# nanograv/PTMCMCSampler

Measured on AMD Instinct MI355X. Metric: MH updates/sec (whole node) + ESS/sec, 100-d Gaussian, 64 temps x 4096 walkers per GPU, higher is better.
Workload: dtype f64

## Files before the change

ptmcmcsampler_amd/csrc/ptmi_abi.hip:

```cpp
#include <math.h>
#include <stdlib.h>

#include <new>
#include <vector>

#include <type_traits>

#include "ptmi_common.h"

static thread_local char g_err[512] = "";
int ptmi_fail(int code, const char *fmt, ...)
{
    va_list ap;
    va_start(ap, fmt);
    vsnprintf(g_err, sizeof(g_err), fmt, ap);
    va_end(ap);
    return code;
}

constexpr int WT = 7, WTILE = 16 * WT;
template <bool FUSED>
__global__ __launch_bounds__(256) void welford_kernel(const double *AM, double *mu, double *M2, double *cov, int d, int mem,
                                                     long long iter, int cov_stride_per_walker, int am_epl)
{
// ... 848 lines not shown
{
    __shared__ int32_t local[GJ_BUCKETS], base[GJ_BUCKETS];
    for (int b = (int)threadIdx.x; b < GJ_BUCKETS; b += (int)blockDim.x) local[b] = 0;
    __syncthreads();
    const long long ch = (long long)blockIdx.x * blockDim.x + threadIdx.x;
    const int b = ch < nch ? gj_class(gj, (size_t)(ch / nt) * nt + temp_of[ch]) : 0;
    const int mine = ch < nch ? atomicAdd(&local[b], 1) : 0;
    __syncthreads();
    for (int bb = (int)threadIdx.x; bb < GJ_BUCKETS; bb += (int)blockDim.x)
        base[bb] = local[bb] ? atomicAdd(&bucket[2 * GJ_BUCKETS + bb], local[bb]) : 0;
    __syncthreads();
    if (ch >= nch) return;
    const long long t = bucket[GJ_BUCKETS + b] + base[b] + mine;
    if (t < nsolo) { order[t * cpw] = (int32_t)ch; return; }
    const long long tr = t - nsolo, nrest = nch - nsolo;
    const long long nw = nrest / cpw, whole = nw * cpw;
    order[(long long)nsolo * cpw + (tr < whole ? (tr % nw) * cpw + tr / nw : tr)] = (int32_t)ch;
}

__global__ void selftest_math_kernel(int op, const double *in, const double *in2, double *out, long long n)
{
    const long long i = (long long)blockIdx.x * blockDim.x + threadIdx.x;
    if (i >= n) return;
    const double x = in[i];
    double r;
    switch (op) {
    case 0: r = det_log(x); break;
    case 1: r = det_exp(x); break;
    case 2: r = det_cos2pi(x); break;
    case 3: r = det_sqrt(x); break;
    case 4: r = x / in2[i]; break;
    case 5: r = det_normal((u64)__double_as_longlong(x), (u64)__double_as_longlong(in2[i])); break;
    case 10: r = unit_log((u64)__double_as_longlong(x)); break;
    case 11: case 12: {
        u32 j;
        double t, sn, cs;
        unit_angle64((u64)__double_as_longlong(x), j, t);
        unit_sincos(j, t, sn, cs);
        r = op == 11 ? cs : sn;
        break;
    }
    case 13: {
        u32 j;
        double t, sn, cs;
        unit_angle32((u32)(u64)__double_as_longlong(x), j, t);
        unit_sincos(j, t, sn, cs);
        r = det_sqrt(-2.0 * unit_log((u64)__double_as_longlong(in2[i]))) * cs;
        break;
    }
    default: r = group_sum<16>(x); break;
    }
    out[i] = r;
}
__global__ void selftest_philox_kernel(const u32 *ck, u32 *out, long long n)
{
    const long long i = (long long)blockIdx.x * blockDim.x + threadIdx.x;
    if (i >= n) return;
    const u32 *c = ck + i * 6;
    u64 w0, w1;
    philox_words(((u64)c[5] << 32) | c[4], ((u64)c[1] << 32) | c[0], c[2], c[3], w0, w1);
    out[i * 4 + 0] = (u32)w0; out[i * 4 + 1] = (u32)(w0 >> 32);
    out[i * 4 + 2] = (u32)w1; out[i * 4 + 3] = (u32)(w1 >> 32);
}

struct Shape { int G, EPL; };
static bool pick_shape(int d, bool grad, Shape *s)
{
    static const Shape table[] = {
#define PTMI_TABLE_ENTRY(G_, E_) {G_, E_},
        PTMI_SHAPE_LIST(PTMI_TABLE_ENTRY)};
    if (d > PTMI_GJ_REG_MAX) grad = false;
    const int G = grad ? ptmi_lanes_for_grad(d) : ptmi_lanes_for(d);
    for (const Shape &c : table)
        if (c.G == G && c.G * c.EPL >= d && (!grad || c.EPL <= 8) && (!ptmi_shape_exact(c.G, c.EPL) || c.G * c.EPL == d)) { *s = c; return true; }
    return false;
}

static KArgs make_args(ptmi_engine *h)
{
    KArgs a;
    memset(&a, 0, sizeof(a));
    a.box_off = -1;
    a.tab_off = -1;
    const ptmi_config &c = h->cfg;
    const ptmi_buffers &b = h->buf;
    a.X = b.X; a.lnL = b.lnL; a.lp = b.lp; a.temp_of = b.temp_of; a.slot_of = b.slot_of;
    a.Ut = b.Ut; a.S = b.S; a.DE = b.DE; a.AM = c.temp0 == 0 ? b.AM : nullptr; a.AMaux = c.temp0 == 0 ? b.AMaux : nullptr;
    a.AMflag = c.temp0 == 0 ? (AmFlag *)b.AMflag : nullptr;
    a.rp_draws = h->rp_draws;
    a.nacc = (u64 *)b.nacc; a.jstat = (u64 *)b.jstat; a.cjstat = h->cjstat;
    a.temps_mh = h->d_temps; a.beta = h->d_beta; a.logl_par = h->d_loglpar; a.logp_par = h->d_logppar;
    a.gsize = h->d_gsize; a.gmask = h->d_gmask; a.gcn = h->d_gcn; a.gdiv = h->d_gdiv; a.ngroups = c.ngroups > 1 ? c.ngroups : 1;
    a.Q = b.Q; a.qaux = b.qaux; a.Q2 = nullptr; a.sloc = nullptr; a.q_cur = 0; a.q_tgt = 0;
    a.seed = c.seed;
    a.d = c.ndim; a.nt = c.ntemps; a.W = c.nwalkers; a.ntg = c.ntemps_global; a.temp0 = c.temp0; a.walker0 = c.walker0;
    a.w_host = c.w_host; a.w_scam = c.w_scam; a.w_am = c.w_am; a.w_de = c.w_de; a.de_on = h->de_on; a.de_size = c.de_size; a.de_head = h->de_head;
    a.cov_update = c.cov_update; a.tskip = c.tskip; a.per_walker = c.cov_per_walker; a.logp_kind = c.logp_kind;
    a.pick_walker = c.pick_mode == PTMI_PICK_WALKER;
    a.de_ld = h->G == 4 ? 8 * ((h->EPL + 1) / 2) : c.ndim;
    a.lanes = h->G;
    a.am_epl = am_row_epl(h->G, h->EPL);
    a.w_nuts = c.w_nuts; a.w_hmc = c.w_hmc; a.gj_nburn = c.gj_nburn; a.hmc_min = c.hmc_min; a.hmc_max = c.hmc_max;
    a.nuts_maxdepth = c.nuts_maxdepth; a.hmc_eps = c.hmc_eps; a.nuts_delta = c.nuts_delta;
    a.gj_tab = h->d_gj_tab; a.gj_diag = h->gj_diag; a.gj = b.gj; a.gj_scr = h->d_gj_scr; a.gj_scal = h->d_gj_scal;
    return a;
}

static ptmi_shape_fn shape_fn(int G, int EPL, int L)
{
    if (L == PTMI_LOGL_INTERVAL) {
#define PTMI_PICK_SHAPE3(G_, E_) if (G == G_ && EPL == E_) return ptmi_shape_##G_##_##E_##_3;
        PTMI_GJ_SHAPE_LIST(PTMI_PICK_SHAPE3)
        return nullptr;
    }
#define PTMI_PICK_SHAPE(G_, E_)                                                                        \
    if (G == G_ && EPL == E_) return L == 0 ? ptmi_shape_##G_##_##E_##_0 : (L == 1 ? ptmi_shape_##G_##_##E_##_1 : ptmi_shape_##G_##_##E_##_2);
    PTMI_SHAPE_LIST(PTMI_PICK_SHAPE)
    return nullptr;
}
static int run_shape(ptmi_engine *h, int op, KArgs &a, int grid, bool full)
{
    const int L = (op == PTMI_OP_PROPOSE || op == PTMI_OP_ACCEPT) ? 0 : h->cfg.logl_kind;
    ptmi_shape_fn f = shape_fn(h->G, h->EPL, L);
    if (!f) return fail(PTMI_EUNSUPPORTED, "no kernel shape for ndim=%d", h->cfg.ndim);
    return f(op, h, a, grid, full);
}

static int set_step_args(const ptmi_engine *h, KArgs *a)
{
    const ptmi_config &c = h->cfg;
    a->am_row0 = (int)(a->iter0 % c.cov_update);
    if (a->AMflag != nullptr && a->nsteps > 0 && (a->iter0 - 1) / c.cov_update != (a->iter0 + a->nsteps - 2) / c.cov_update && a->iter0 > 0)
        return fail(PTMI_EINVAL, "with AM row flags a launch may not cross a multiple of cov_update (iterations %lld..%lld, cov_update=%d)",
                    a->iter0, a->iter0 + a->nsteps - 1, c.cov_update);
    a->swap_last = 0;
    if (c.tskip > 0 && c.ntemps_global > 1) {
        const long long last = a->iter0 + a->nsteps - 1;
        if (last / c.tskip != (a->iter0 - 1) / c.tskip && last % c.tskip != 0)
            return fail(PTMI_EINVAL, "iterations %lld..%lld contain a swap iteration (Tskip=%d) before their end", a->iter0, last, c.tskip);
        if ((last / c.tskip) - ((a->iter0 - 1) / c.tskip) > 1)
            return fail(PTMI_EINVAL, "iterations %lld..%lld span more than one swap epoch", a->iter0, last);
        a->swap_last = last % c.tskip == 0;
    }
    return PTMI_OK;
}

static int chains_grid(const ptmi_engine *h)
{
    const long long nch = (long long)h->cfg.nwalkers * h->cfg.ntemps;
    const int cpb = 256 / h->G;
    return (int)((nch + cpb - 1) / cpb);
}

template <int G, int MAXT>
static int launch_am_gemm_t(ptmi_engine *h, long long max_events)
{
    const size_t lds = sizeof(double) * 2 * (2 * G) * 64;
    auto kern = am_gemm_kernel<G, MAXT>;
    if (lds > 64 * 1024) {
        hipError_t e = hipFuncSetAttribute((const void *)kern, hipFuncAttributeMaxDynamicSharedMemorySize, (int)lds);
        if (e != hipSuccess) return fail(PTMI_EHIP, "hipFuncSetAttribute(%zu B of LDS): %s", lds, hipGetErrorString(e));
    }
    const int d = h->cfg.ndim, ntile = (d + 15) / 16, parts = (ntile + 4 * MAXT - 1) / (4 * MAXT);
    const int ngr = h->cfg.ngroups > 1 ? h->cfg.ngroups : 1;
    const int pw = h->cfg.cov_per_walker ? 1 : 0;
    const long long per_key = pw ? (max_events / h->cfg.nwalkers) : max_events;
// ... 892 lines not shown
```

ptmcmcsampler_amd/csrc/ptmi_common.h:

```cpp
#pragma once
#include <hip/hip_runtime.h>
#include <stdarg.h>
#include <stdio.h>
#include <stdlib.h>
#include <string.h>

#include "../../include/ptmi.h"
#include "ptmi_device.h"

using namespace ptmi;

int ptmi_fail(int code, const char *fmt, ...);
#define fail ptmi_fail
inline double ptmi_env(const char *name, double dflt)
{
    const char *v = getenv(name);
    return v ? strtod(v, nullptr) : dflt;
}

#define HIPCHK(expr)                                                                          \
    do {                                                                                      \
        hipError_t e_ = (expr);                                                               \
        if (e_ != hipSuccess) return fail(PTMI_EHIP, "%s: %s (%s:%d)", #expr, hipGetErrorString(e_), __FILE__, __LINE__); \
    } while (0)

__host__ __device__ inline int am_pos(int i, int epl)
{
    if (epl == 0) return i;
    const int e = i >> 2, ln = i & 3;
    return e < 2 * (epl / 2) ? 8 * (e >> 1) + 2 * ln + (e & 1) : 8 * (epl / 2) + ln;
}
__host__ __device__ inline int am_inv(int p, int epl)
{
    if (epl == 0) return p;
    const int h = 8 * (epl / 2);
    return p < h ? ((p & 7) >> 1) + 4 * (2 * (p >> 3) + (p & 1)) : (p - h) + 4 * (epl - 1);
}
constexpr int am_row_epl(int G, int EPL) { return (G == 4 && EPL == 25) ? EPL : 0; }

constexpr unsigned long long AMROW_NEW = 1ull;
constexpr unsigned long long AMROW_KEY = 2ull;
typedef unsigned long long AmFlag;

struct KArgs {
    double *X, *lnL, *lp;
    int32_t *temp_of, *slot_of;
    const double *Ut, *S, *DE;
    double *AM, *AMaux;
    AmFlag *AMflag;
    u64 *nacc, *jstat;
    const double *temps_mh, *beta, *logl_par, *logp_par;
    const int32_t *gsize;
    const double *gmask, *gcn, *gdiv;
    double *Q, *qaux;
    double *Q2;
    int32_t *sloc;
    int q_cur, q_tgt;
    const double *newlnL, *newlp;
    u64 seed;
    long long iter0;
    const long long *iter_dev;
    int nsteps;
    int d, nt, W, ntg, temp0, walker0;
    int w_host, w_scam, w_am, w_de, de_on, de_size, de_head;
    int cov_update, tskip, per_walker, logp_kind, ngroups;
    int am_row0, swap_last;
    int am_epl;
    int lanes;
    int de_ld;
    int pick_walker;
    int lds_u;
    int amq_off;
    int amq_on;
    int box_off;
    int tab_off;
    const double *am_inc;
    const long long *am_base;
    long long *am_next;
    const double *UtPad;
    int ut_pad_ld;
    const double *ut_absmax;
    int umax_off;
    int w_nuts, w_hmc, gj_nburn, hmc_min, hmc_max, nuts_maxdepth;
    double hmc_eps, nuts_delta;
    const double *gj_tab;
    int gj_diag;
    double *gj;
    double *gj_scr, *gj_scal;
    int gj_stack_off, gj_lds_levels;
    const int32_t *gj_order;
    int gj_nslots;
    const u64 *rp_draws;
    u64 *cjstat;
};

enum { GJ_EPS = 0, GJ_MU = 1, GJ_HBAR = 2, GJ_EPSBAR = 3, GJ_NITER = 4, GJ_HITER = 5, GJ_HAVE_EPS = 6, GJ_NLEAP = 7 , GJ_NSTATE = 8 };
constexpr int GJ_BUCKETS = 128;
constexpr u32 SLOT_GJ = 0x2000000u;
constexpr u32 SLOT_GJS = 0x3000000u;
constexpr u32 SLOT_CJ = 0x4000000u;
constexpr int PTMI_CJ_MAXFUN = 32;
enum { GJV_TM = 0, GJV_RM = 1, GJV_GM = 2, GJV_TP = 3, GJV_RP = 4, GJV_GP = 5, GJV_SAMPLE = 6, GJV_TOP = 7 };
enum { GJL_FAR_T = 0, GJL_FAR_R = 1, GJL_CAND_T = 2, GJL_CAND_G = 3, GJL_VECS = 4 };
enum { GJS_LOGP = 0, GJS_N = 1, GJS_ALPHA = 2, GJS_NALPHA = 3, GJS_SCALARS = 4 };

constexpr int PTMI_GJ_REG_MAX = 512;

template <int G>
__device__ __forceinline__ double group_bcast_lane(double v, int src)
{
    const int lane = (int)(threadIdx.x & 63);
    return __shfl(v, (lane & ~(G - 1)) + src, 64);
}

struct ptmi_engine {
    ptmi_config cfg;
    ptmi_buffers buf;
    hipStream_t stream;
    double *d_ladder, *d_temps, *d_beta, *d_loglpar, *d_logppar, *d_gmask, *d_gcn, *d_gdiv;
    int32_t *d_gsize;
    void *d_pre;
    int32_t *d_hop;
    bool hop_from_sweep;
    int32_t *h_hop;
    hipEvent_t hop_ev;
    bool hop_pending;
    int32_t *d_xint;
    double *d_gj_tab, *d_gj_scr, *d_gj_scal;
    int gj_diag;
    int gj_solo;
    int32_t *d_gj_order, *d_gj_bucket;
    void *d_am_ev;
    int32_t *d_am_count;
    long long *d_am_base;
    double *d_am_inc;
    int32_t *d_am_grp, *d_am_perm;
    long long *d_am_kbase;
    long long am_cap;
    int am_piece;
    double *d_pool_part, *d_pool_T;
    int G, EPL;
    int de_on, de_head;
    int last_variant;
    hipEvent_t ev0, ev1;
    hipStream_t side;
    hipEvent_t side_go, side_done;
    double *d_utpad;
    void *d_sy_scr;
    void *dc_plan;
    int32_t *h_sy_info;
    void *d_qlg_scr;
    int32_t *gsize_host;
    void *d_ql_scr;
    void *d_qlw_scr;
    size_t qlw_scr_bytes;
    void *d_rle_ent;
    int32_t *d_rle_cnt;
    const double *rp_swap_u;
    const u64 *rp_draws;
    long long *d_am_next;
    int split_am_piece;
    long long split_am_lo, split_am_hi;
    long long *d_iter;
    int dev_iter;
    int q_cur;
    int gj_phase;
    long long gj_iter, gj_n;
    void *gj_work;
    long long *h_gj_n;
    u64 *cjstat;
    int32_t *d_cj_fun;
    int cj_nfun, cj_phase;
    long long cj_iter;
    void *cj_work;
    long long cj_offs[PTMI_CJ_MAXFUN + 1];
    long long *h_cj_offs;
// ... 35 lines not shown
```

ptmcmcsampler_amd/csrc/ptmi_mh.inc.h:

```cpp
#pragma once
#include <stdlib.h>

#include "ptmi_common.h"

template <bool STR, int J>
__device__ __forceinline__ u64 grp_bcast(u64 v)
{
    if (STR) return (u64)__shfl((long long)v, (int)(threadIdx.x & 15) + 16 * J, 64);
    return quad_bcast<J>(v);
}
template <bool STR, int J>
__device__ __forceinline__ double grp_bcastf(double v)
{
    if (STR) return __shfl(v, (int)(threadIdx.x & 15) + 16 * J, 64);
    return quad_bcastf<J>(v);
}
template <int G, bool STR>
__device__ __forceinline__ double grp_sum(double p)
{
    if (STR) {
        p = p + __shfl_xor(p, 32, 64);
        p = p + __shfl_xor(p, 16, 64);
        return p;
    }
// ... 859 lines not shown
                for (int e = 0; e < EPL; e += 2) {
                    double wa, wb;
                    weights(e, wa, wb);
                    wk[e] = wa;
                    if (e + 1 < EPL) wk[e + 1] = wb;
                    __builtin_amdgcn_sched_barrier(0);
                }
#pragma unroll
                for (int e = 0; e < EPL; ++e) dq[e] = 0.0;
#pragma unroll
                for (int e2 = 0; e2 < EPL; ++e2) {
#pragma unroll 1
                    for (int src = 0; src < G; ++src) {
                        const int k = src + G * e2;
                        if (k >= ng) break;
                        const double wv = group_bcast_lane<G>(wk[e2], src);
                        const double *row = Ut + (size_t)k * d;
#pragma unroll
                        for (int e = 0; e < EPL; ++e) {
                            double r;
                            PTMI_ROW_LOAD_S(PSAFE, r, row, e);
                            dq[e] = __builtin_fma(r, wv, dq[e]);
                        }
                    }
                }
            }
        }
    };
    if (jt == PTMI_J_SCAM) scam_body();
    else if (FULL && jt == PTMI_J_DE) de_body();
    if (FULL && am_here && (!STR ? is_am : __any(is_am))) am_body();
    return jt;
}

template <int G, int EPL>
__device__ __forceinline__ void am_store_row(double *am, const double (&x)[EPL], int gl, int d)
{
    if constexpr (am_row_epl(G, EPL) != 0) {
        ptmi_d2 *ap = reinterpret_cast<ptmi_d2 *>(am) + gl;
#pragma unroll
        for (int e2 = 0; e2 < EPL / 2; ++e2) __builtin_nontemporal_store(ptmi_d2{x[2 * e2], x[2 * e2 + 1]}, &ap[4 * e2]);
        if (EPL & 1) __builtin_nontemporal_store(x[EPL - 1], &am[8 * (EPL / 2) + gl]);
    } else {
#pragma unroll
        for (int e = 0; e < EPL; ++e) {
            const int i = gl + G * e;
            if (e < safe_slots(G, EPL) || i < d) __builtin_nontemporal_store(x[e], &am[i]);
        }
    }
}

template <int G, int EPL>
__device__ __forceinline__ void am_store_step(const KArgs &a, int w, int am_row, int k, const double (&x)[EPL], int gl, int d, bool accepted)
{
    const size_t r = (size_t)w * a.cov_update + (size_t)am_row;
    if (a.AMflag != nullptr) {
        const bool key = k == 0 || am_row <= 1;
        if (gl == 0) __builtin_nontemporal_store((key ? AMROW_KEY : 0ull) | (accepted ? AMROW_NEW : 0ull), a.AMflag + r);
        if (!(key || accepted)) return;
    }
    am_store_row<G, EPL>(a.AM + r * d, x, gl, d);
}

__device__ __forceinline__ int logical_block()
{
    const int nb = (int)gridDim.x, b = (int)blockIdx.x;
    return (nb & 7) == 0 ? (b & 7) * (nb >> 3) + (b >> 3) : b;
}

#ifndef PTMI_WIDE_MINBLK
#define PTMI_WIDE_MINBLK 0
#endif
constexpr int mh_min_blocks(int G, int EPL, int LOGL, bool FULL, bool STAGE, bool GRP, int PERS, bool UPAD, int PRI)
{
#ifndef PTMI_GRPFULL_MINBLK
#define PTMI_GRPFULL_MINBLK 2
#endif
    if (FULL && GRP && !STAGE && !PERS && G == 4 && LOGL != PTMI_LOGL_DENSE) return PTMI_GRPFULL_MINBLK;
    if (PERS || STAGE || FULL || LOGL == PTMI_LOGL_DENSE) return 1;
    if (UPAD && PRI == PTMI_LOGP_FLAT && LOGL == PTMI_LOGL_ISO) return PTMI_WIDE_MINBLK ? PTMI_WIDE_MINBLK : (EPL <= 16 ? 4 : (EPL <= 26 ? 3 : 2));
    if (UPAD && PRI == PTMI_LOGP_BOX && LOGL == PTMI_LOGL_ISO) return EPL <= 16 ? 3 : 2;
    return 2;
}
template <int G, int EPL, int LOGL, bool FULL, bool STAGE, bool GRP, bool ULDS = false, int PERS = 0, int PRI = -1 ,
          bool TLDS = false ,
          bool UPAD = false >
__global__ __launch_bounds__(PERS ? PERS : 256, mh_min_blocks(G, EPL, LOGL, FULL, STAGE, GRP, PERS, UPAD, PRI)) void mh_steps_kernel(const KArgs a)
{
    static_assert(!UPAD || (G > 4 && !FULL && !STAGE && !GRP && !ULDS), "UPAD is a variant of the wide SCAM-only kernel");
    static_assert(!ULDS || (!STAGE && !FULL && !GRP), "ULDS is the SCAM-only contiguous-layout kernel");
    static_assert(!PERS || (ULDS && G == 4), "persistent blocks are a variant of the ULDS kernel");
    constexpr int TM = (STAGE && FULL) ? 2 : 0;
    constexpr int BLK = PERS ? PERS : 256;
    constexpr int CPB = BLK / G;
    constexpr bool STR = STAGE;
    const int d = a.d, nt = a.nt;
    const long long nch = (long long)a.W * nt;
    const int lane = (int)(threadIdx.x & 63), wave = (int)(threadIdx.x >> 6);
    const int cib = STR ? wave * 16 + (lane & 15) : (int)(threadIdx.x / G);
    const int gl = STR ? lane >> 4 : (int)(threadIdx.x % G);
    extern __shared__ __attribute__((aligned(16))) double smem[];
    constexpr bool SCAMFAST = !FULL && !GRP;
    constexpr bool BOXFAST = SCAMFAST && PRI == PTMI_LOGP_BOX && UPAD && G == 64;
    constexpr bool PAIRED = ULDS && G == 4 && EPL == 25;
    constexpr int LD = mfma_ld(EPL);
    const int tab_n = 4 * ((d + 3) / 4) * LD;
    const double *PtG = LOGL == PTMI_LOGL_DENSE ? a.logl_par + d + (size_t)d * d : nullptr;
#define PTMI_PL (smem)
#define PTMI_UL (smem + (LOGL == PTMI_LOGL_DENSE ? (size_t)tab_n : 0))
#define PTMI_SQ (smem + (size_t)tab_n * ((LOGL == PTMI_LOGL_DENSE ? 1 : 0) + ((UT_ALWAYS_LDS || a.lds_u) ? 1 : 0)))
    constexpr bool UT_ALWAYS_LDS = LOGL != PTMI_LOGL_DENSE;
    const double *const tsm = TM ? smem : nullptr;
    size_t w0 = 0;
    if (!PERS && a.per_walker) {
        const long long ch0 = (long long)logical_block() * CPB;
        w0 = (size_t)((ch0 < nch ? ch0 : nch - 1) / nt);
    }
    const double *const UtBlk = a.Ut + w0 * d * d;
    if (TM) draw_table_fill(smem, a.tab_off, BLK);
    if (STAGE) {
        if (LOGL == PTMI_LOGL_DENSE) {
            for (int i = (int)threadIdx.x; i < tab_n; i += BLK) {
                const int r = i / LD, c = i % LD;
                PTMI_PL[i] = (r < d && c < d) ? PtG[(size_t)r * d + c] : 0.0;
            }
        }
        if (FULL) {
            const double *Sb = a.S + w0 * d;
            for (int i = (int)threadIdx.x; i < d; i += BLK) PTMI_SQ[i] = det_sqrt(Sb[i]);
        }
        if (FULL && (UT_ALWAYS_LDS || a.lds_u)) {
            for (int i = (int)threadIdx.x; i < tab_n; i += BLK) {
                const int r = i / LD, c = i % LD;
                PTMI_UL[i] = (r < d && c < d) ? UtBlk[(size_t)r * d + c] : 0.0;
            }
        }
        __syncthreads();
    }
    const bool ulds_box = ULDS && !PERS && a.logp_kind == PTMI_LOGP_BOX && a.box_off >= 0 && a.box_off < d * d + d;
    if (ULDS) {
        const double *src = UtBlk, *srcS = a.S + w0 * d;
        if constexpr (PAIRED) {
            auto perm = [](int c) { const int ln = c & 3, e = c >> 2; return e < 2 * (EPL / 2) ? 8 * (e >> 1) + 2 * ln + (e & 1) : 8 * (EPL / 2) + ln; };
            if (d == 4 * EPL) {
                constexpr int NPAIR = 2 * EPL * 4 * EPL, NB = 10;
                const ptmi_d2 *src2 = reinterpret_cast<const ptmi_d2 *>(src);
                for (int base = 0; base < NPAIR; base += NB * BLK) {
                    ptmi_d2 tmp[NB];
#pragma unroll
                    for (int u = 0; u < NB; ++u) {
                        const int idx = base + (int)threadIdx.x + u * BLK;
                        tmp[u] = src2[idx < NPAIR ? idx : NPAIR - 1];
                    }
#pragma unroll
                    for (int u = 0; u < NB; ++u) {
                        const int idx = base + (int)threadIdx.x + u * BLK;
                        if (idx < NPAIR) {
                            const int r = (2 * idx) / (4 * EPL), c = (2 * idx) % (4 * EPL);
                            smem[r * (4 * EPL) + perm(c)] = tmp[u].x;
                            smem[r * (4 * EPL) + perm(c + 1)] = tmp[u].y;
                        }
                    }
                }
            } else {
                for (int i = (int)threadIdx.x; i < d * d; i += BLK) {
                    const int r = i / d, c = i % d;
                    smem[r * d + perm(c)] = src[i];
                }
            }
        } else {
            for (int i = (int)threadIdx.x; i < d * d; i += BLK) smem[i] = src[i];
        }
        if (!ulds_box)
            for (int i = (int)threadIdx.x; i < d; i += BLK) smem[d * d + i] = det_sqrt(srcS[i]);
    }
    if (PRI != PTMI_LOGP_FLAT) box_table_fill<G, EPL>(a, smem, BLK);
    if (ULDS) draw_table_fill(smem, a.tab_off, BLK);
    if constexpr (BOXFAST && PERS != 0) {
        if (threadIdx.x == 0) reinterpret_cast<unsigned long long *>(smem)[a.umax_off] = 0ull;
    }
    if (ULDS || (a.logp_kind == PTMI_LOGP_BOX && a.box_off >= 0)) __syncthreads();
    double box_umax = 0.0;
    if constexpr (BOXFAST) {
        if constexpr (PERS != 0) {
            double am = 0.0;
            for (int i = (int)threadIdx.x; i < d * d; i += BLK) { const double v = __builtin_fabs(smem[i]); am = v > am ? v : am; }
            __hip_atomic_fetch_max(reinterpret_cast<unsigned long long *>(smem) + a.umax_off, (unsigned long long)__double_as_longlong(am), __ATOMIC_RELAXED,
                                   __HIP_MEMORY_SCOPE_WORKGROUP);
            __syncthreads();
            box_umax = smem[a.umax_off];
        } else {
            box_umax = *a.ut_absmax;
        }
        box_umax *= 1.0 + 0x1.0p-30;
    }

    const long long nunits = (nch + 15) / 16, ustride = PERS ? (long long)gridDim.x * (BLK / 64) : nunits;
    const int upw = nt / 16, upw1 = upw > 1 ? upw - 1 : 1;
    const bool cold_first = PERS && a.AM != nullptr && a.temp0 == 0 && nt % 16 == 0;
    for (long long upos = PERS ? (long long)blockIdx.x * (BLK / 64) + wave : 0; upos < nunits; upos += ustride) {
    long long unit = upos;
    if (cold_first) {
        const long long r = upos - a.W;
        const int wq = upos < a.W ? (int)upos : (int)(r / upw1);
        const int cq = __builtin_amdgcn_readfirstlane(a.slot_of[(size_t)wq * nt]) >> 4;
        unit = (long long)wq * upw + (upos < a.W ? cq : (cq + 1 + (int)(r % upw1)) % upw);
    }
    long long ch = PERS ? unit * 16 + (STR ? (lane & 15) : (lane >> 2)) : (long long)logical_block() * CPB + cib;
    const bool live = ch < nch;
    if (!live) ch = nch - 1;
    const int w = (int)(ch / nt);
    const int t = a.temp_of[ch];
    const int tg = a.temp0 + t;
    const double beta = a.beta[t];
    const ChainConst cc = chain_const(a.temps_mh[t], beta, d);
    const u32 sid0 = (u32)((u64)(a.walker0 + w) * (u32)a.ntg);
    const u32 sid = sid0 + (u32)tg;
    const size_t wc = a.per_walker ? (size_t)w : 0;
    const double *Ut = a.Ut + wc * a.ngroups * d * d, *S = a.S + wc * a.ngroups * d;
    const double *DE = (FULL && a.DE) ? a.DE + wc * (size_t)a.de_size * a.de_ld : nullptr;
    double *xrow = a.X + (size_t)ch * d;
    constexpr int GW = (G > 4 && !STR && !ULDS) ? G : 4;
    DrawBatch<STR, GW> batch;
    ScamBatch<STR, GW> sbatch;
    const double *UtBlock = (STAGE && FULL) ? UtBlk : Ut;

    constexpr bool AMQ = STAGE && FULL && G == 4;
    constexpr int AMQ_LD = 4 * EPL + 2;
#define PTMI_AMQ(slot) (smem + a.amq_off + ((size_t)wave * 16 + (size_t)(slot)) * AMQ_LD)
#define PTMI_AMQ_IDX ((int *)(smem + a.amq_off + (size_t)4 * 16 * AMQ_LD) + wave * 128)
    const bool amq_on = AMQ && a.amq_on;
    u64 mask_c = 0, mask_n = 0;
    int rank_c = 0, rank_n = 0, base_c = 0, base_n = 0, q_done = 0;
    double cd_c = 0.0, cd_n = 0.0;

    constexpr bool PIPE = PAIRED && PERS != 0 && !FULL && !GRP && LOGL == PTMI_LOGL_ISO && PRI == PTMI_LOGP_FLAT;
    double x[EPL], dq[EPL], urow[PIPE ? EPL : 1];
#pragma unroll
    for (int e = 0; e < EPL; ++e) PTMI_ROW_LOAD(x[e], xrow, e);
    double lnL = a.lnL[ch], lp = a.lp[ch];
    u32 nacc = 0, jp[PTMI_J_FUSED] = {0, 0, 0}, ja[PTMI_J_FUSED] = {0, 0, 0};
    long long am_next = (FULL && a.am_base != nullptr) ? a.am_base[ch] : 0;
    const bool cold = live && tg == 0 && a.AM != nullptr;
    int am_row = a.am_row0;
    double box_margin = -1.0;
    double box_guard = 0.0;

    constexpr bool SQUAD = SCAMFAST && ScamBatch<STR, GW>::QUAD;
    constexpr bool PASSES = GW > 4 || SQUAD;
    constexpr int KPASS = GW > 4 ? GW / 2 : (SQUAD ? 4 : (1 << 30));
    constexpr int STM = (PERS || TLDS) ? 1 : (ULDS ? 2 : 0);
    auto scam_root_s = [&](int kk) {
        if (ULDS && !ulds_box) return smem[d * d + kk];
        return det_sqrt(S[kk]);
    };
    [[maybe_unused]] int koff = 0;
    [[maybe_unused]] auto row_request = [&](int off) __attribute__((always_inline)) {
        if constexpr (PIPE) {
            const double *row = smem + off;
            const ptmi_d2 *rp = reinterpret_cast<const ptmi_d2 *>(row) + gl;
#pragma unroll
            for (int e2 = 0; e2 < EPL / 2; ++e2) { const ptmi_d2 v = rp[4 * e2]; urow[2 * e2] = v.x; urow[2 * e2 + 1] = v.y; }
            if (EPL & 1) urow[EPL - 1] = row[8 * (EPL / 2) + gl];
        }
    };
    int kp = 0;
    if constexpr (PIPE) {
        for (; a.nsteps - kp >= 4; kp += 4) {
            sbatch.template refill<STM>(a, a.iter0 + kp, sid, gl, cc, d, [&](int kk) {
                const double rs = scam_root_s(kk);
                koff = kk * d;
                row_request((int)dpp32<0x00>((u32)koff));
                __builtin_amdgcn_sched_barrier(0);
                return rs;
            }, smem);
            {
                const int k = kp;
#define PTMI_STEP_S 0
#include "ptmi_mh_step.inc.h"
#undef PTMI_STEP_S
            }
            {
                const int k = kp + 1;
#define PTMI_STEP_S 1
#include "ptmi_mh_step.inc.h"
#undef PTMI_STEP_S
            }
            {
                const int k = kp + 2;
#define PTMI_STEP_S 2
#include "ptmi_mh_step.inc.h"
#undef PTMI_STEP_S
            }
            {
                const int k = kp + 3;
#define PTMI_STEP_S 3
#include "ptmi_mh_step.inc.h"
#undef PTMI_STEP_S
            }
        }
    }
    for (int k0 = PIPE ? kp : 0; k0 < a.nsteps; k0 += KPASS) {
    const int kend = (PASSES && a.nsteps - k0 > KPASS) ? k0 + KPASS : a.nsteps;
    if constexpr (GW > 4) {
        if constexpr (SCAMFAST) sbatch.template refill<0>(a, a.iter0 + k0, sid, gl, cc, d, [&](int kk) { return det_sqrt(S[kk]); }, nullptr);
        else batch.template refill<TM>(a, a.iter0 + k0, sid, gl, tsm);
    } else if constexpr (SQUAD) {
        sbatch.template refill<STM>(a, a.iter0 + k0, sid, gl, cc, d, scam_root_s, smem);
    }
    for (int k = k0; k < kend; ++k) {
#define PTMI_STEP_S (-1)
#include "ptmi_mh_step.inc.h"
#undef PTMI_STEP_S
    }
    }
    if (live) {
#pragma unroll
        for (int e = 0; e < EPL; ++e) {
            const int i = gl + G * e;
            if (e < safe_slots(G, EPL) || i < d) xrow[i] = x[e];
        }
        if (gl == 0) {
            a.lnL[ch] = lnL;
            a.lp[ch] = lp;
            const size_t r = (size_t)w * nt + t;
            a.nacc[r] += nacc;
            if (!FULL) { jp[PTMI_J_SCAM] = (u32)a.nsteps; ja[PTMI_J_SCAM] = nacc; }
#pragma unroll
            for (int j = 0; j < PTMI_J_FUSED; ++j) {
                a.jstat[(r * PTMI_J_NTYPES + j) * 2 + 0] += jp[j];
                a.jstat[(r * PTMI_J_NTYPES + j) * 2 + 1] += ja[j];
            }
        }
    }
    }
}

#ifndef PTMI_PC_PRIO
#define PTMI_PC_PRIO 0
#endif
#ifndef PTMI_PC_SPRIO
#define PTMI_PC_SPRIO 1
#endif
#ifndef PTMI_PC_ACCV
#define PTMI_PC_ACCV 1
#endif
#ifndef PTMI_PC_SLEEP
#define PTMI_PC_SLEEP 2
#endif
template <int EPL, int LOGL, int PRI, bool PERS>
__global__ __launch_bounds__(512) void mh_pc_kernel(const KArgs a)
{
    constexpr int G = 4, CPB = 64;
    constexpr bool STR = true;
    constexpr int LD = mfma_ld(EPL), AMQ_LD = 4 * EPL + 2;
    constexpr bool DENSE = LOGL == PTMI_LOGL_DENSE;
    const int d = a.d, nt = a.nt;
    const long long nch = (long long)a.W * nt;
    const int lane = (int)(threadIdx.x & 63), wave8 = (int)(threadIdx.x >> 6);
    const int pair = wave8 & 3;
    const bool producer = wave8 >= 4;
    const int c16 = lane & 15, gl = lane >> 4;
    extern __shared__ __attribute__((aligned(16))) double smem[];
    const int tab_n = 4 * ((d + 3) / 4) * LD;
#define PTMI_PC_UL (smem)
#define PTMI_PC_SQ (smem + (size_t)tab_n)
#define PTMI_PC_RING(slot) (smem + a.amq_off + ((size_t)pair * 16 + (size_t)(slot)) * AMQ_LD)
#define PTMI_PC_CD (smem + a.amq_off + (size_t)4 * 16 * AMQ_LD + (size_t)pair * 128)
#define PTMI_PC_IDX ((int *)(smem + a.amq_off + (size_t)4 * 16 * AMQ_LD + (size_t)4 * 128) + pair * 128)
#define PTMI_PC_FLG ((int *)(smem + a.amq_off + (size_t)4 * 16 * AMQ_LD + (size_t)4 * 128) + 4 * 128 + pair * 2)
#define PTMI_PC_MU (smem + a.amq_off + (size_t)4 * 16 * AMQ_LD + (size_t)4 * 128 + 260)
    size_t w0 = 0;
    if (!PERS && a.per_walker) {
        const long long ch0 = (long long)logical_block() * CPB;
        w0 = (size_t)((ch0 < nch ? ch0 : nch - 1) / nt);
    }
    {
        const double *UtBlk = a.Ut + w0 * d * d, *Sb = a.S + w0 * d;
        const double *src = DENSE ? a.logl_par + d + (size_t)d * d  : UtBlk;
        draw_table_fill(smem, a.tab_off, 512);
        for (int i = (int)threadIdx.x; i < d; i += 512) PTMI_PC_SQ[i] = det_sqrt(Sb[i]);
        for (int i = (int)threadIdx.x; i < tab_n; i += 512) {
            const int r = i / LD, c = i % LD;
            PTMI_PC_UL[i] = (r < d && c < d) ? src[(size_t)r * d + c] : 0.0;
        }
        box_table_fill<G, EPL>(a, smem, 512);
        if (threadIdx.x < 8) ((int *)(smem + a.amq_off + (size_t)4 * 16 * AMQ_LD + (size_t)4 * 128) + 4 * 128)[threadIdx.x] = 0;
        if constexpr (DENSE)
            for (int i = (int)threadIdx.x; i < 4 * EPL; i += 512) PTMI_PC_MU[i] = i < d ? a.logl_par[i] : 0.0;
        __syncthreads();
    }
    const long long nunits = (nch + 15) / 16;
    const long long ustride = PERS ? (long long)gridDim.x * 4 : nunits;
    int *const flg = PTMI_PC_FLG;
    const double *const UtG = a.Ut + w0 * d * d;
    if (producer) {
        if (PTMI_PC_PRIO) __builtin_amdgcn_s_setprio(PTMI_PC_PRIO);
        const int w_de = a.de_on ? a.w_de : 0;
        const u32 L = (u32)(a.w_host + a.w_scam + a.w_am + w_de);
        int known = 0, q_done = 0;
        int *const idx = PTMI_PC_IDX;
        double *const cdl = PTMI_PC_CD;
        for (long long unit = (long long)(PERS ? blockIdx.x : logical_block()) * 4 + pair; unit < nunits; unit += ustride) {
            long long ch = unit * 16 + c16;
            const bool live = ch < nch;
            if (!live) ch = nch - 1;
            const int w = (int)(ch / nt);
            const int t = a.temp_of[ch];
            const ChainConst cc = chain_const(a.temps_mh[t], a.beta[t], d);
            const u32 sid0 = (u32)((u64)(a.walker0 + w) * (u32)a.ntg);
            const u32 sid = sid0 + (u32)(a.temp0 + t);
            int kb = 0;
            for (;;) {
                while (known - q_done < 16 && kb < a.nsteps) {
                    bool ev = false;
                    double cdv = 0.0;
                    if (kb + gl < a.nsteps) {
                        u64 p0, p1;
// ... 503 lines not shown
                    hipError_t e = hipFuncSetAttribute((const void *)kern, hipFuncAttributeMaxDynamicSharedMemorySize, (int)lds2);
                    if (e != hipSuccess) return fail(PTMI_EHIP, "hipFuncSetAttribute(%zu B of LDS): %s", lds2, hipGetErrorString(e));
                }
                const int cpb = 512 / G;
                hipLaunchKernelGGL(kern, dim3((unsigned)((nch + cpb - 1) / cpb)), dim3(512), lds2, h->stream, a);
                h->last_variant = PTMI_VAR_STAGED | PTMI_VAR_LDS_UT | PTMI_VAR_DENSE_SCAM | (a.box_off >= 0 ? PTMI_VAR_LDS_BOX : 0);
                return PTMI_OK;
            };
            if (c.logp_kind == PTMI_LOGP_BOX) return launch(mh_dense_scam_kernel<EPL, 512, true>);
            return launch(mh_dense_scam_kernel<EPL, 512, false>);
        }
    }
    if constexpr (WANTS) {
        const size_t tab = sizeof(double) * (size_t)(4 * ((c.ndim + 3) / 4)) * mfma_ld(EPL);
        const bool one_table_per_block = c.ngroups <= 1 && (!FULL || !c.cov_per_walker || c.ntemps % (256 / G) == 0);
        size_t lds = LOGL == PTMI_LOGL_DENSE ? tab : 0;
        const bool dense_pc = FULL && LOGL == PTMI_LOGL_DENSE && EPL >= 14 && c.w_am > 0 && one_table_per_block && !ptmi_env("PTMI_NO_PC", 0);
        if (FULL && !dense_pc && lds + tab + sizeof(double) * c.ndim <= 160 * 1024) { a.lds_u = 1; lds += tab; }
        if (FULL) lds += sizeof(double) * c.ndim;
        const size_t amq = FULL ? sizeof(double) * 4 * 16 * (4 * EPL + 2) + sizeof(int) * 4 * 128 : 0;
        if (sizeof(double) * even(lds / sizeof(double)) + amq <= 160 * 1024 && one_table_per_block) {
            if (FULL) {
                a.amq_off = (int)even(lds / sizeof(double));
                lds = sizeof(double) * (size_t)a.amq_off + amq;
                const int Lw = c.w_host + c.w_scam + c.w_am + (h->de_on ? c.w_de : 0);
                const double f = Lw > 0 ? (double)c.w_am / (double)Lw : 0.0;
                a.amq_on = c.pick_mode != PTMI_PICK_WALKER && c.w_am > 0 && 1.28 * f < 1.0 - pow(1.0 - f, 16.0);
            }
            if (box_bytes && sizeof(double) * even(lds / sizeof(double)) + box_bytes <= 160 * 1024) {
                a.box_off = (int)even(lds / sizeof(double));
                lds = sizeof(double) * (size_t)a.box_off + box_bytes;
            }
            if (FULL && sizeof(double) * even(lds / sizeof(double)) + DRAWT <= 160 * 1024) {
                a.tab_off = (int)even(lds / sizeof(double));
                lds = sizeof(double) * (size_t)a.tab_off + DRAWT;
            }
            if constexpr (FULL) {
                const bool no_pc = ptmi_env("PTMI_NO_PC", 0) != 0;
                const size_t lists = sizeof(double) * 4 * 128 + sizeof(int) * 8 + (LOGL == PTMI_LOGL_DENSE ? sizeof(double) * 4 * EPL : 0);
                const bool tables_ok = LOGL == PTMI_LOGL_DENSE ? !a.lds_u : a.lds_u != 0;
                if (c.w_am > 0 && tables_ok && a.tab_off >= 0 && !no_pc && lds + lists <= 160 * 1024 &&
                    (c.logp_kind == PTMI_LOGP_FLAT || (c.logp_kind == PTMI_LOGP_BOX && a.box_off >= 0))) {
                    const int shift = (int)(lists / sizeof(double));
                    if (a.box_off >= 0) a.box_off += shift;
                    a.tab_off += shift;
                    const size_t ldp = lds + lists;
                    static int ncu = 0;
                    if (!ncu && (hipDeviceGetAttribute(&ncu, hipDeviceAttributeMultiprocessorCount, c.device) != hipSuccess || ncu < 1)) ncu = 256;
                    const bool pers = !c.cov_per_walker;
                    const int gridp = pers ? (grid < ncu ? grid : ncu) : grid;
                    auto launch_pc = [&](auto kp) -> int {
                        if (ldp > 64 * 1024) {
                            hipError_t e = hipFuncSetAttribute((const void *)kp, hipFuncAttributeMaxDynamicSharedMemorySize, (int)ldp);
                            if (e != hipSuccess) return fail(PTMI_EHIP, "hipFuncSetAttribute(%zu B of LDS): %s", ldp, hipGetErrorString(e));
                        }
                        hipLaunchKernelGGL(kp, dim3(gridp), dim3(512), ldp, h->stream, a);
                        h->last_variant = PTMI_VAR_STAGED | PTMI_VAR_FULL | (a.lds_u ? PTMI_VAR_LDS_UT : 0) | PTMI_VAR_PC |
                                          (a.box_off >= 0 ? PTMI_VAR_LDS_BOX : 0) | PTMI_VAR_LDS_DRAWT | (pers ? PTMI_VAR_PERSISTENT : 0);
                        return PTMI_OK;
                    };
                    if (pers) {
                        if (c.logp_kind == PTMI_LOGP_BOX) return launch_pc(mh_pc_kernel<EPL, LOGL, PTMI_LOGP_BOX, true>);
                        return launch_pc(mh_pc_kernel<EPL, LOGL, PTMI_LOGP_FLAT, true>);
                    }
                    if (c.logp_kind == PTMI_LOGP_BOX) return launch_pc(mh_pc_kernel<EPL, LOGL, PTMI_LOGP_BOX, false>);
                    return launch_pc(mh_pc_kernel<EPL, LOGL, PTMI_LOGP_FLAT, false>);
                }
            }
            auto kern = mh_steps_kernel<G, EPL, LOGL, FULL, true, false>;
            if (lds > 64 * 1024) {
                hipError_t e = hipFuncSetAttribute((const void *)kern, hipFuncAttributeMaxDynamicSharedMemorySize, (int)lds);
                if (e != hipSuccess) return fail(PTMI_EHIP, "hipFuncSetAttribute(%zu B of LDS): %s", lds, hipGetErrorString(e));
            }
            hipLaunchKernelGGL(kern, dim3(grid), dim3(256), lds, h->stream, a);
            h->last_variant = PTMI_VAR_STAGED | (FULL ? PTMI_VAR_FULL : 0) | (a.lds_u ? PTMI_VAR_LDS_UT : 0) | (a.amq_on ? PTMI_VAR_AMQ : 0) |
                              (a.box_off >= 0 ? PTMI_VAR_LDS_BOX : 0) | (a.tab_off >= 0 ? PTMI_VAR_LDS_DRAWT : 0);
            return PTMI_OK;
        }
    }
    if constexpr (!FULL && LOGL != PTMI_LOGL_DENSE) {
        size_t tab = sizeof(double) * ((size_t)c.ndim * c.ndim + c.ndim);
        const bool one_table = c.ngroups <= 1 && (!c.cov_per_walker || c.ntemps % (256 / G) == 0);
        if constexpr (G == 4) {
            if (c.ngroups <= 1 && !c.cov_per_walker && ptmi_env("PTMI_ULDS_PERS", 1) && (c.logp_kind == PTMI_LOGP_FLAT || c.logp_kind == PTMI_LOGP_BOX)) {
                static int ncu = 0;
                if (!ncu) {
                    if (hipDeviceGetAttribute(&ncu, hipDeviceAttributeMultiprocessorCount, c.device) != hipSuccess || ncu < 1) ncu = 256;
                }
                size_t tp = sizeof(double) * even((size_t)c.ndim * c.ndim + c.ndim);
                a.box_off = -1;
                if (box_bytes) { a.box_off = (int)(tp / sizeof(double)); tp += box_bytes; }
                a.tab_off = (int)(tp / sizeof(double));
                tp += DRAWT;
                a.umax_off = (int)(tp / sizeof(double));
                tp += 16;
                auto launch_p = [&](auto kernp, int BLKv) -> int {
                    if (tp > 64 * 1024) {
                        hipError_t e = hipFuncSetAttribute((const void *)kernp, hipFuncAttributeMaxDynamicSharedMemorySize, (int)tp);
                        if (e != hipSuccess) return fail(PTMI_EHIP, "hipFuncSetAttribute(%zu B of LDS): %s", tp, hipGetErrorString(e));
                    }
                    const long long nunits = ((long long)c.nwalkers * c.ntemps + 15) / 16, wpb = BLKv / 64;
                    const long long nb = (nunits + wpb - 1) / wpb;
                    hipLaunchKernelGGL(kernp, dim3((unsigned)(nb < ncu ? nb : ncu)), dim3(BLKv), tp, h->stream, a);
                    h->last_variant = PTMI_VAR_LDS_UT | PTMI_VAR_PERSISTENT | (a.box_off >= 0 ? PTMI_VAR_LDS_BOX : 0) | PTMI_VAR_LDS_DRAWT;
                    return PTMI_OK;
                };
                if (tp <= 160 * 1024) {
                    if (c.logp_kind == PTMI_LOGP_BOX) return launch_p(mh_steps_kernel<G, EPL, LOGL, false, false, false, true, 512, PTMI_LOGP_BOX>, 512);
                    return launch_p(mh_steps_kernel<G, EPL, LOGL, false, false, false, true, 512, PTMI_LOGP_FLAT>, 512);
                }
                a.box_off = -1;
                a.tab_off = -1;
            }
        }
        if (box_bytes) {
            const size_t ut = sizeof(double) * even((size_t)c.ndim * c.ndim);
            if (2 * (sizeof(double) * even(tab / sizeof(double)) + box_bytes) <= 160 * 1024) {
                a.box_off = (int)even(tab / sizeof(double));
                tab = sizeof(double) * (size_t)a.box_off + box_bytes;
            } else if (2 * (ut + box_bytes) <= 160 * 1024) {
                a.box_off = (int)(ut / sizeof(double));
                tab = ut + box_bytes;
            }
        }
        if (one_table && 2 * tab <= 160 * 1024) {
            if (2 * (sizeof(double) * even(tab / sizeof(double)) + DRAWT) <= 160 * 1024) {
                a.tab_off = (int)even(tab / sizeof(double));
                tab = sizeof(double) * (size_t)a.tab_off + DRAWT;
            }
            auto launch_u = [&](auto kern) -> int {
                if (tab > 64 * 1024) {
                    hipError_t e = hipFuncSetAttribute((const void *)kern, hipFuncAttributeMaxDynamicSharedMemorySize, (int)tab);
                    if (e != hipSuccess) return fail(PTMI_EHIP, "hipFuncSetAttribute(%zu B of LDS): %s", tab, hipGetErrorString(e));
                }
                hipLaunchKernelGGL(kern, dim3(grid), dim3(256), tab, h->stream, a);
                return PTMI_OK;
            };
            if (int rc = a.tab_off >= 0 ? launch_u(mh_steps_kernel<G, EPL, LOGL, false, false, false, true, 0, -1, true>)
                                        : launch_u(mh_steps_kernel<G, EPL, LOGL, false, false, false, true>)) return rc;
            h->last_variant = PTMI_VAR_LDS_UT | (a.box_off >= 0 ? PTMI_VAR_LDS_BOX : 0) | (a.tab_off >= 0 ? PTMI_VAR_LDS_DRAWT : 0);
            return PTMI_OK;
        }
    }
    a.box_off = box_bytes ? 0 : -1;
    if constexpr (G > 4 && !FULL) {
        if (a.UtPad != nullptr && a.ut_pad_ld == G * EPL && c.ngroups <= 1) {
            if (c.logp_kind == PTMI_LOGP_FLAT)
                hipLaunchKernelGGL((mh_steps_kernel<G, EPL, LOGL, false, false, false, false, 0, PTMI_LOGP_FLAT, false, true>), dim3(grid), dim3(256), 0, h->stream, a);
            else if (G == 64 && c.logp_kind == PTMI_LOGP_BOX && a.ut_absmax != nullptr)
                hipLaunchKernelGGL((mh_steps_kernel<G, EPL, LOGL, false, false, false, false, 0, PTMI_LOGP_BOX, false, true>), dim3(grid), dim3(256), box_bytes, h->stream, a);
            else
                hipLaunchKernelGGL((mh_steps_kernel<G, EPL, LOGL, false, false, false, false, 0, -1, false, true>), dim3(grid), dim3(256), box_bytes, h->stream, a);
            h->last_variant = PTMI_VAR_UTPAD | (a.box_off >= 0 ? PTMI_VAR_LDS_BOX : 0);
            return PTMI_OK;
        }
    }
    if (c.ngroups > 1) hipLaunchKernelGGL((mh_steps_kernel<G, EPL, LOGL, FULL, false, true>), dim3(grid), dim3(256), box_bytes, h->stream, a);
    else hipLaunchKernelGGL((mh_steps_kernel<G, EPL, LOGL, FULL, false, false>), dim3(grid), dim3(256), box_bytes, h->stream, a);
    h->last_variant = (FULL ? PTMI_VAR_FULL : 0) | (c.ngroups > 1 ? PTMI_VAR_GROUPS : 0) | (a.box_off >= 0 ? PTMI_VAR_LDS_BOX : 0);
    return PTMI_OK;
}
```

Baseline: 35.28 billion.

## Precompute per-wave unit plans and per-temperature chain constants in LDS for persistent kernel

In the persistent MH kernel, each wave now resolves its next batch of up to 8 work units at once (cold-first unit mapping, walker base, and per-chain temperature index) and writes them into an LDS plan table. Per-temperature constants (beta and chain_const outputs) are computed once per block into LDS instead of being recomputed per chain per unit. This targets the scattered global loads of temp_of, slot_of and beta and the chain_const arithmetic in the unit loop's critical path. In exchange it uses extra LDS, adds loop nesting, and limits the launch path to chain counts below 2^30.

```diff
diff --git a/ptmcmcsampler_amd/csrc/ptmi_abi.hip b/ptmcmcsampler_amd/csrc/ptmi_abi.hip
--- a/ptmcmcsampler_amd/csrc/ptmi_abi.hip
+++ b/ptmcmcsampler_amd/csrc/ptmi_abi.hip
@@ -954,6 +954,9 @@
     memset(&a, 0, sizeof(a));
     a.box_off = -1;
     a.tab_off = -1;
+    a.plan_off = -1;
+    a.cc_off = -1;
+    a.plan_p = 1;
     const ptmi_config &c = h->cfg;
     const ptmi_buffers &b = h->buf;
     a.X = b.X; a.lnL = b.lnL; a.lp = b.lp; a.temp_of = b.temp_of; a.slot_of = b.slot_of;
diff --git a/ptmcmcsampler_amd/csrc/ptmi_common.h b/ptmcmcsampler_amd/csrc/ptmi_common.h
--- a/ptmcmcsampler_amd/csrc/ptmi_common.h
+++ b/ptmcmcsampler_amd/csrc/ptmi_common.h
@@ -92,6 +92,7 @@
     int gj_nslots;
     const u64 *rp_draws;
     u64 *cjstat;
+    int plan_off, cc_off, plan_p;
 };
 
 enum { GJ_EPS = 0, GJ_MU = 1, GJ_HBAR = 2, GJ_EPSBAR = 3, GJ_NITER = 4, GJ_HITER = 5, GJ_HAVE_EPS = 6, GJ_NLEAP = 7 , GJ_NSTATE = 8 };
diff --git a/ptmcmcsampler_amd/csrc/ptmi_mh.inc.h b/ptmcmcsampler_amd/csrc/ptmi_mh.inc.h
--- a/ptmcmcsampler_amd/csrc/ptmi_mh.inc.h
+++ b/ptmcmcsampler_amd/csrc/ptmi_mh.inc.h
@@ -965,6 +965,7 @@
     if (UPAD && PRI == PTMI_LOGP_BOX && LOGL == PTMI_LOGL_ISO) return EPL <= 16 ? 3 : 2;
     return 2;
 }
+constexpr int PLAN_UNITS = 8, PLAN_ENTRY = 18, CC_ENTRY = 8;
 template <int G, int EPL, int LOGL, bool FULL, bool STAGE, bool GRP, bool ULDS = false, int PERS = 0, int PRI = -1 ,
           bool TLDS = false ,
           bool UPAD = false >
@@ -1021,6 +1022,47 @@
         __syncthreads();
     }
     const bool ulds_box = ULDS && !PERS && a.logp_kind == PTMI_LOGP_BOX && a.box_off >= 0 && a.box_off < d * d + d;
+    constexpr bool planned = PERS != 0;
+    const long long p_nunits = planned ? (nch + 15) / 16 : 0, p_ustride = planned ? (long long)gridDim.x * (BLK / 64) : 0;
+    const int p_upw = planned ? nt / 16 : 0, p_upw1 = p_upw > 1 ? p_upw - 1 : 1;
+    const bool p_cold_first = planned && a.AM != nullptr && a.temp0 == 0 && nt % 16 == 0;
+#define PTMI_PLAN (reinterpret_cast<int *>(smem + a.plan_off) + wave * (PLAN_UNITS * PLAN_ENTRY))
+    [[maybe_unused]] auto plan_resolve = [&](unsigned upos0) -> unsigned {
+        unsigned pos = upos0 + (unsigned)(lane & (PLAN_UNITS - 1)) * (unsigned)p_ustride;
+        if (pos >= (unsigned)p_nunits) pos = (unsigned)p_nunits - 1u;
+        unsigned unit = pos;
+        if (p_cold_first) {
+            const unsigned W = (unsigned)a.W, r = pos - W;
+            const bool cu = pos < W;
+            const unsigned wq = cu ? pos : r / (unsigned)p_upw1;
+            const unsigned cq = (unsigned)a.slot_of[(size_t)wq * nt] >> 4;
+            unit = wq * (unsigned)p_upw + (cu ? cq : (cq + 1u + r % (unsigned)p_upw1) % (unsigned)p_upw);
+        }
+        return unit;
+    };
+    [[maybe_unused]] auto plan_write = [&](unsigned unit_l) {
+        const unsigned last = (unsigned)(nch - 1), c = (unsigned)(lane & 15);
+        int tw[PLAN_UNITS / 4];
+        unsigned un[PLAN_UNITS / 4], w0[PLAN_UNITS / 4];
+#pragma unroll
+        for (int h = 0; h < PLAN_UNITS / 4; ++h) {
+            un[h] = (unsigned)__shfl((int)unit_l, 4 * h + (lane >> 4), 64);
+            const unsigned c0 = un[h] * 16u < last ? un[h] * 16u : last, chp = un[h] * 16u + c < last ? un[h] * 16u + c : last;
+            w0[h] = c0 / (unsigned)nt;
+            tw[h] = a.temp_of[chp] | (int)((chp / (unsigned)nt - w0[h]) << 24);
+        }
+#pragma unroll
+        for (int h = 0; h < PLAN_UNITS / 4; ++h) {
+            int *pe = PTMI_PLAN + (4 * h + (lane >> 4)) * PLAN_ENTRY;
+            pe[2 + c] = tw[h];
+            if (c == 0) { pe[0] = (int)un[h]; pe[1] = (int)w0[h]; }
+        }
+    };
+    const long long upos_first = planned ? (long long)blockIdx.x * (BLK / 64) + wave : 0;
+    [[maybe_unused]] unsigned plan_unit0 = 0;
+    if constexpr (planned) {
+        if (upos_first < p_nunits) plan_unit0 = plan_resolve((unsigned)upos_first);
+    }
     if (ULDS) {
         const double *src = UtBlk, *srcS = a.S + w0 * d;
         if constexpr (PAIRED) {
@@ -1059,6 +1101,15 @@
     }
     if (PRI != PTMI_LOGP_FLAT) box_table_fill<G, EPL>(a, smem, BLK);
     if (ULDS) draw_table_fill(smem, a.tab_off, BLK);
+    if constexpr (planned) {
+        if (upos_first < p_nunits) plan_write(plan_unit0);
+        for (int r = (int)threadIdx.x; r < nt; r += BLK) {
+            const double b = a.beta[r];
+            const ChainConst c = chain_const(a.temps_mh[r], b, d);
+            double *ce = smem + a.cc_off + (size_t)CC_ENTRY * r;
+            ce[0] = b; ce[1] = c.cd0; ce[2] = c.cd1; ce[3] = c.cd2; ce[4] = c.sc0; ce[5] = c.sc1; ce[6] = c.sc2; ce[7] = c.de_mul;
+        }
+    }
     if constexpr (BOXFAST && PERS != 0) {
         if (threadIdx.x == 0) reinterpret_cast<unsigned long long *>(smem)[a.umax_off] = 0ull;
     }
@@ -1081,22 +1132,48 @@
     const long long nunits = (nch + 15) / 16, ustride = PERS ? (long long)gridDim.x * (BLK / 64) : nunits;
     const int upw = nt / 16, upw1 = upw > 1 ? upw - 1 : 1;
     const bool cold_first = PERS && a.AM != nullptr && a.temp0 == 0 && nt % 16 == 0;
-    for (long long upos = PERS ? (long long)blockIdx.x * (BLK / 64) + wave : 0; upos < nunits; upos += ustride) {
+    [[maybe_unused]] const int plan_p = planned ? a.plan_p : 1;
+    [[maybe_unused]] long long ubase = upos_first;
+    do {
+    if constexpr (planned) {
+        if (ubase != upos_first) {
+            asm volatile("" ::: "memory");
+            plan_write(plan_resolve((unsigned)ubase));
+            asm volatile("" ::: "memory");
+        }
+    }
+    [[maybe_unused]] int pi = 0;
+    for (long long upos = PERS ? ubase : 0; upos < nunits && (!planned || pi < plan_p); upos += ustride, ++pi) {
+    [[maybe_unused]] long long p_ch = 0;
+    [[maybe_unused]] int p_w = 0, p_t = 0;
+    [[maybe_unused]] double p_beta = 0.0;
+    [[maybe_unused]] ChainConst p_cc = {};
+    if constexpr (planned) {
+        const int *pe = PTMI_PLAN + pi * PLAN_ENTRY;
+        const int p_unit = __builtin_amdgcn_readfirstlane(pe[0]), w0p = __builtin_amdgcn_readfirstlane(pe[1]);
+        const int tw = pe[2 + (lane >> 2)];
+        p_ch = (long long)p_unit * 16 + (lane >> 2);
+        p_w = w0p + (tw >> 24);
+        p_t = tw & 0xffffff;
+        const double *ce = smem + a.cc_off + (size_t)CC_ENTRY * p_t;
+        p_beta = ce[0];
+        p_cc.cd0 = ce[1]; p_cc.cd1 = ce[2]; p_cc.cd2 = ce[3]; p_cc.sc0 = ce[4]; p_cc.sc1 = ce[5]; p_cc.sc2 = ce[6]; p_cc.de_mul = ce[7];
+    }
     long long unit = upos;
-    if (cold_first) {
+    if (!planned && cold_first) {
         const long long r = upos - a.W;
         const int wq = upos < a.W ? (int)upos : (int)(r / upw1);
         const int cq = __builtin_amdgcn_readfirstlane(a.slot_of[(size_t)wq * nt]) >> 4;
         unit = (long long)wq * upw + (upos < a.W ? cq : (cq + 1 + (int)(r % upw1)) % upw);
     }
-    long long ch = PERS ? unit * 16 + (STR ? (lane & 15) : (lane >> 2)) : (long long)logical_block() * CPB + cib;
+    long long ch = planned ? p_ch : (PERS ? unit * 16 + (STR ? (lane & 15) : (lane >> 2)) : (long long)logical_block() * CPB + cib);
     const bool live = ch < nch;
     if (!live) ch = nch - 1;
-    const int w = (int)(ch / nt);
-    const int t = a.temp_of[ch];
+    const int w = planned ? p_w : (int)(ch / nt);
+    const int t = planned ? p_t : a.temp_of[ch];
     const int tg = a.temp0 + t;
-    const double beta = a.beta[t];
-    const ChainConst cc = chain_const(a.temps_mh[t], beta, d);
+    const double beta = planned ? p_beta : a.beta[t];
+    const ChainConst cc = planned ? p_cc : chain_const(a.temps_mh[t], beta, d);
     const u32 sid0 = (u32)((u64)(a.walker0 + w) * (u32)a.ntg);
     const u32 sid = sid0 + (u32)tg;
     const size_t wc = a.per_walker ? (size_t)w : 0;
@@ -1217,6 +1294,8 @@
         }
     }
     }
+        ubase += plan_p * ustride;
+    } while (planned && ubase < nunits);
 }
 
 #ifndef PTMI_PC_PRIO
@@ -1886,7 +1965,8 @@
         size_t tab = sizeof(double) * ((size_t)c.ndim * c.ndim + c.ndim);
         const bool one_table = c.ngroups <= 1 && (!c.cov_per_walker || c.ntemps % (256 / G) == 0);
         if constexpr (G == 4) {
-            if (c.ngroups <= 1 && !c.cov_per_walker && ptmi_env("PTMI_ULDS_PERS", 1) && (c.logp_kind == PTMI_LOGP_FLAT || c.logp_kind == PTMI_LOGP_BOX)) {
+            if (c.ngroups <= 1 && !c.cov_per_walker && ptmi_env("PTMI_ULDS_PERS", 1) && (c.logp_kind == PTMI_LOGP_FLAT || c.logp_kind == PTMI_LOGP_BOX) &&
+                (long long)c.nwalkers * c.ntemps < (1ll << 30) && c.ntemps < (1 << 24)) {
                 static int ncu = 0;
                 if (!ncu) {
                     if (hipDeviceGetAttribute(&ncu, hipDeviceAttributeMultiprocessorCount, c.device) != hipSuccess || ncu < 1) ncu = 256;
@@ -1898,6 +1978,13 @@
                 tp += DRAWT;
                 a.umax_off = (int)(tp / sizeof(double));
                 tp += 16;
+                a.plan_off = (int)even(tp / sizeof(double));
+                a.cc_off = a.plan_off + (int)((size_t)(512 / 64) * PLAN_UNITS * PLAN_ENTRY * sizeof(int) / sizeof(double));
+                tp = sizeof(double) * ((size_t)a.cc_off + (size_t)CC_ENTRY * c.ntemps);
+                {
+                    const double pv = ptmi_env("PTMI_ULDS_PERS", 1);
+                    a.plan_p = (pv >= 2 && pv <= 1 + PLAN_UNITS) ? (int)pv - 1 : PLAN_UNITS;
+                }
                 auto launch_p = [&](auto kernp, int BLKv) -> int {
                     if (tp > 64 * 1024) {
                         hipError_t e = hipFuncSetAttribute((const void *)kernp, hipFuncAttributeMaxDynamicSharedMemorySize, (int)tp);
@@ -1915,6 +2002,7 @@
                 }
                 a.box_off = -1;
                 a.tab_off = -1;
+                a.plan_off = a.cc_off = -1;
             }
         }
         if (box_bytes) {
```

Result: no change. 35.60 billion, median of 6 (+0.9%).
